# simonsobs/pixell

Measured on AMD Instinct MI355X. Metric: map2alm+alm2map round-trips/sec, higher is better.
Workload: dtype f64

## Files before the change

pixell_amd/csrc/leg_s0.hip:

```cpp
#include "legendre_dev.hpp"

namespace pxs {

#define S0_SYN_PAIR(c0, c1, a0, a1) { \
	PXS_VCOPY(vb0, polar ? c0.c : c0.b); \
	PXS_VCOPY(vb1, polar ? c1.c : c1.b); \
	_Pragma("unroll") for (int s = 0; s < K; s++) { \
		p1r[s] = fma(lam2[s], a0.a, p1r[s]); p1i[s] = fma(lam2[s], a0.b, p1i[s]); \
		p2r[s] = fma(lam2[s], a0.c, p2r[s]); p2i[s] = fma(lam2[s], a0.d, p2i[s]); \
		lam1[s] = fma(fma(c0.a, csq[s], vb0), lam2[s], lam1[s]); \
	} \
	_Pragma("unroll") for (int s = 0; s < K; s++) { \
		p1r[s] = fma(lam1[s], a1.a, p1r[s]); p1i[s] = fma(lam1[s], a1.b, p1i[s]); \
		p2r[s] = fma(lam1[s], a1.c, p2r[s]); p2i[s] = fma(lam1[s], a1.d, p2i[s]); \
		lam2[s] = fma(fma(c1.a, csq[s], vb1), lam1[s], lam2[s]); \
	} }

template<int K> __global__ __launch_bounds__(64, (K == 4 ? 7 : 1)) void leg_syn_s0(const LegK a)
{
	const int lane = threadIdx.x; int wv, m, bb;
	if (!leg_block(a, wv, m, bb)) return;
	const long row0 = PXS_UNIFORM_LONG(a.row[m]);
	const int nk = (a.lmax - m)/2 + 1;
	const double4_t* __restrict__ coef = a.coef + row0;
// ... 33 lines not shown
#pragma unroll
			for (int s = 0; s < K; s++)
				if (sc[s] < 0 && fabs(lam2[s]) > SC_BIG) {
					lam1[s] *= SC_SMALL; lam2[s] *= SC_SMALL;
					if (++sc[s] == 0) p1r[s] = p1i[s] = p2r[s] = p2i[s] = 0;
				}
		}
#pragma unroll
		for (int s = 0; s < K; s++) if (sc[s] < 0) { p1r[s] = p1i[s] = p2r[s] = p2i[s] = 0; lam1[s] = lam2[s] = 0; }
		double4_t c0 = LDC(coef, k), c1 = LDC(coef, k+1), a0 = LDC(at, k), a1 = LDC(at, k+1);
#ifndef PXS_NO_PHASEC_UNROLL
		while (k + 3 < nk) {
			double4_t n0 = LDC(coef, k+2), n1 = LDC(coef, k+3), m0 = LDC(at, k+2), m1 = LDC(at, k+3);
			S0_SYN_PAIR(c0, c1, a0, a1)
			k += 2;
			c0 = LDC(coef, k+2); c1 = LDC(coef, k+3); a0 = LDC(at, k+2); a1 = LDC(at, k+3);
			S0_SYN_PAIR(n0, n1, m0, m1)
			k += 2;
		}
#endif
		for (; k + 1 < nk; k += 2) {
			const double4_t n0 = LDC(coef, k+2), n1 = LDC(coef, k+3), m0 = LDC(at, k+2), m1 = LDC(at, k+3);
			S0_SYN_PAIR(c0, c1, a0, a1)
			c0 = n0; c1 = n1; a0 = m0; a1 = m1;
		}
		if (k < nk) {
#pragma unroll
			for (int s = 0; s < K; s++) {
				p1r[s] = fma(lam2[s], a0.a, p1r[s]); p1i[s] = fma(lam2[s], a0.b, p1i[s]);
				p2r[s] = fma(lam2[s], a0.c, p2r[s]); p2i[s] = fma(lam2[s], a0.d, p2i[s]);
			}
		}
	}
	double2* __restrict__ out = a.leg + (long)bb*a.leg_bs + (long)m*a.ld;
#pragma unroll
	for (int s = 0; s < K; s++) {
		const int p = (wv*K + s)*64 + lane;
		const bool valid = p < a.npairs;
		const int rn_ = valid ? a.ring_n[p] : -1, rs_ = valid ? a.ring_s[p] : -1;
		const double x_ = valid ? a.cth[p] : 0.0;
		if (rn_ >= 0) out[rn_] = make_double2(p1r[s] + x_*p2r[s], p1i[s] + x_*p2i[s]);
		if (rs_ >= 0) out[rs_] = make_double2(p1r[s] - x_*p2r[s], p1i[s] - x_*p2i[s]);
	}
}

#define S0_ANA_PAIR(c0, c1) { \
	PXS_VCOPY(vb0, polar ? c0.c : c0.b); \
	PXS_VCOPY(vb1, polar ? c1.c : c1.b); \
	double t0 = 0, t1 = 0, t2 = 0, t3 = 0, u0 = 0, u1 = 0, u2 = 0, u3 = 0; \
	_Pragma("unroll") for (int s = 0; s < K; s++) { \
		t0 = fma(lam2[s], d1r[s], t0); t1 = fma(lam2[s], d1i[s], t1); t2 = fma(lam2[s], d2r[s], t2); t3 = fma(lam2[s], d2i[s], t3); \
		lam1[s] = fma(fma(c0.a, csq[s], vb0), lam2[s], lam1[s]); \
	} \
	_Pragma("unroll") for (int s = 0; s < K; s++) { \
		u0 = fma(lam1[s], d1r[s], u0); u1 = fma(lam1[s], d1i[s], u1); u2 = fma(lam1[s], d2r[s], u2); u3 = fma(lam1[s], d2i[s], u3); \
		lam2[s] = fma(fma(c1.a, csq[s], vb1), lam1[s], lam2[s]); \
	} \
	 \
	LEG_RED_PUT(kk, t0, t1, t2, t3) \
	LEG_RED_PUT(kk+1, u0, u1, u2, u3) \
	kk += 2; \
	if (kk == LEG_FSTEPS) { leg_flush(red, pout + 4*kbase, lane, LEG_FSTEPS, a.atomic); kk = 0; kbase = k+2; } }

template<int K> __global__ __launch_bounds__(64) void leg_ana_s0(const LegK a)
{
	PXS_SHARED(double, red);
	const int lane = threadIdx.x; int wv, m, bb;
	if (!leg_block(a, wv, m, bb)) return;
	const long row0 = PXS_UNIFORM_LONG(a.row[m]);
	const int nk = (a.lmax - m)/2 + 1;
	const double4_t* __restrict__ coef = a.coef + row0;
	double* __restrict__ pout = a.part + (long)bb*a.mom_bs + ((long)wv*a.rows_chunk + (row0 - a.rowbase))*4;
	const double2* __restrict__ in = a.leg + (long)bb*a.leg_bs + (long)m*a.ld;
	double csq[K], lam1[K], lam2[K], d1r[K], d1i[K], d2r[K], d2i[K];
	int sc[K];
	bool alive_any = false;
	const bool polar = leg_wave_polar(a, wv, K);
	auto load_data = [&](int s) {
		const int p = (wv*K + s)*64 + lane;
		const bool valid = p < a.npairs;
		const int rn = valid ? a.ring_n[p] : -1, rs = valid ? a.ring_s[p] : -1;
		const double x = valid ? a.cth[p] : 0.0;
		const double2 vn = rn >= 0 ? in[rn] : make_double2(0, 0);
		const double2 vs = rs >= 0 ? in[rs] : make_double2(0, 0);
		d1r[s] = vn.x + vs.x; d1i[s] = vn.y + vs.y;
		d2r[s] = (vn.x - vs.x)*x; d2i[s] = (vn.y - vs.y)*x;
	};
#pragma unroll
	for (int s = 0; s < K; s++) {
		const int p = (wv*K + s)*64 + lane;
		const bool valid = p < a.npairs;
		const double x = valid ? a.cth[p] : 0.0;
		const double sth = valid ? a.sth[p] : 0.0;
		csq[s] = polar ? -sth*sth : x*x;
		const bool alive = valid && ((double)m <= a.lmax*sth + a.ofs);
		lam1[s] = 0; lam2[s] = 0; sc[s] = 0;
		if (alive && a.seed_mode != 2) { double mt; int e; pow_scaled(sth, m, mt, e); to_scaled(mt, e, lam2[s], sc[s]); }
		d1r[s] = d1i[s] = d2r[s] = d2i[s] = 0;
		alive_any |= alive;
	}
	if (!__any(alive_any)) return;
	int k = 0;
	S0_SEEDED_PHASE_A
	k = PXS_UNIFORM_INT(k); coef = (const double4_t*)PXS_UNIFORM_LONG((long)coef);
	PXS_COUNT(1, (long)(nk - k)*K*6 + (a.seed_mode != 2 ? (long)k*K*2 : 0L));
	if (lane == 0 && !a.atomic) a.first[wv*a.nmc + (m - a.m0)] = k + 1;
#pragma unroll
	for (int s = 0; s < K; s++) if (sc[s] == 0) load_data(s);
	int kk = 0, kbase = k;
	while (k + 1 < nk) {
		bool pend = false;
#pragma unroll
		for (int s = 0; s < K; s++) pend |= (sc[s] < 0);
		if (!__any(pend)) break;
		for (int it = 0; it < 2 && k + 1 < nk; it++, k += 2) {
			const double4_t c0 = LDC(coef, k), c1 = LDC(coef, k+1);
			S0_ANA_PAIR(c0, c1)
		}
#pragma unroll
		for (int s = 0; s < K; s++)
			if (sc[s] < 0 && fabs(lam2[s]) > SC_BIG) {
				lam1[s] *= SC_SMALL; lam2[s] *= SC_SMALL;
				if (++sc[s] == 0) load_data(s);
			}
	}
	double4_t c0 = LDC(coef, k), c1 = LDC(coef, k+1);
#ifndef PXS_NO_PHASEC_UNROLL
	while (k + 3 < nk) {
		double4_t n0 = LDC(coef, k+2), n1 = LDC(coef, k+3);
		S0_ANA_PAIR(c0, c1)
		k += 2;
		c0 = LDC(coef, k+2); c1 = LDC(coef, k+3);
		S0_ANA_PAIR(n0, n1)
		k += 2;
	}
#endif
	for (; k + 1 < nk; k += 2) {
		const double4_t n0 = LDC(coef, k+2), n1 = LDC(coef, k+3);
		S0_ANA_PAIR(c0, c1)
		c0 = n0; c1 = n1;
	}
	if (k < nk) {
		double t0 = 0, t1 = 0, t2 = 0, t3 = 0;
#pragma unroll
		for (int s = 0; s < K; s++) { t0 = fma(lam2[s], d1r[s], t0); t1 = fma(lam2[s], d1i[s], t1); t2 = fma(lam2[s], d2r[s], t2); t3 = fma(lam2[s], d2i[s], t3); }
		LEG_RED_PUT(kk, t0, t1, t2, t3)
		kk++;
	}
	if (kk > 0) leg_flush(red, pout + 4*kbase, lane, kk, a.atomic);
}


#if defined(PXS_LAB_MMTIME) && !defined(PXS_HOST_SIM)
__device__ unsigned long long mm_prof[16];
#define MM_T0 long long tprev_ = clock64(); unsigned long long tacc_[14] = {0, 0, 0, 0, 0, 0, 0, 0, 0, 0, 0, 0, 0, 0};
#define MM_TICK(i) { const long long tn_ = clock64(); tacc_[i] += (unsigned long long)(tn_ - tprev_); tprev_ = tn_; }
#define MM_TDUMP if (lane == 0) { for (int i_ = 0; i_ < 14; i_++) atomicAdd(&mm_prof[i_], tacc_[i_]); atomicAdd(&mm_prof[15], 1ull); }
#else
#define MM_T0
#define MM_TICK(i)
#define MM_TDUMP
#endif
template<int NG, int W> __global__ __launch_bounds__(64*W, 4) void leg_ana_s0_mm(const LegK a)
{
	PXS_SHARED(double, sh);
	constexpr int K = 1;
	MM_T0
	double* __restrict__ ptile = sh;
	double* __restrict__ red = sh + W*16*MM_PSTRIDE;
	int* __restrict__ s_kmin = reinterpret_cast<int*>(sh + mm_lds_doubles(NG, W));
	const int tid = threadIdx.x, lane = tid & 63, w = PXS_UNIFORM_INT(tid >> 6);
	int wv, m, bb;
	if (!leg_block(a, wv, m, bb)) return;
	const long row0 = PXS_UNIFORM_LONG(a.row[m]);
	const int nk = (a.lmax - m)/2 + 1;
	const double4_t* __restrict__ coef = a.coef + row0;
	const int pbase = wv*64*W;
	const bool polar = [&] { const double c = a.cth[min(pbase + 64*(w + 1), a.npairs) - 1]; return c*c > PXS_POLAR_COS2; }();
	double csq[K], lam1[K], lam2[K]; int sc[K];
	bool alive;
	{
		const int p = pbase + tid;
		const bool valid = p < a.npairs;
		const double x = valid ? a.cth[p] : 0.0, sth = valid ? a.sth[p] : 0.0;
		csq[0] = polar ? -sth*sth : x*x;
		alive = valid && ((double)m <= a.lmax*sth + a.ofs);
		lam1[0] = 0; lam2[0] = 0; sc[0] = 0;
		if (alive) { double mt; int e; pow_scaled(sth, m, mt, e); to_scaled(mt, e, lam2[0], sc[0]); }
	}
	if (tid == 0) *s_kmin = nk;
	__syncthreads();
	MM_TICK(0)
	int k = 0;
	const bool wave_alive = __any(alive);
	if (wave_alive) { S0_PHASE_A }
	const int kw = wave_alive ? PXS_UNIFORM_INT(k) : nk + 16;
	MM_TICK(1)
	if (lane == 0) atomicMin(s_kmin, kw);
	__syncthreads();
	const int kmin = PXS_UNIFORM_INT(*s_kmin);
	MM_TICK(2)
// ... 212 lines not shown
				pmine[(4*q4 + 0)*MMS_PSTRIDE + lane] = p0; pmine[(4*q4 + 1)*MMS_PSTRIDE + lane] = p1;
				pmine[(4*q4 + 2)*MMS_PSTRIDE + lane] = p2; pmine[(4*q4 + 3)*MMS_PSTRIDE + lane] = p3;
			}
			MM_WAVE_SYNC();
			double av[4];
#pragma unroll
			for (int rb = 0; rb < 4; rb++) av[rb] = pread[16*rb];
			MM_WAVE_SYNC();
			if (k0 + 16 < nk) {
#pragma unroll
				for (int i = 0; i < 32; i++) cf[i] = LDCD(tab, 2L*(k0 + 16) + i);
				load_b(k0 + 16, bnxt);
			}
#pragma unroll
			for (int q = 0; q < 4; q++)
#pragma unroll
				for (int rb = 0; rb < 4; rb++) {
					const double aq = q == 0 ? av[rb] : pread[q*MMS_PSTRIDE + 16*rb];
#pragma unroll
					for (int g = 0; g < NG; g++) acc[g][rb] = mm_mfma(aq, bcur[g][q], acc[g][rb]);
				}
			MM_WAVE_SYNC();
#pragma unroll
			for (int g = 0; g < NG; g++)
#pragma unroll
				for (int q = 0; q < 4; q++) bcur[g][q] = bnxt[g][q];
		}
	}
	const int c = lane & 3;
#pragma unroll
	for (int g = 0; g < NG; g++) {
		const int map = (bb*NG + g)*4 + ((lane & 15) >> 2);
		double* __restrict__ out = reinterpret_cast<double*>(a.leg + (long)(map < a.nmaps ? map : 0)*a.leg_bs + (long)m*a.ld) + (c & 1);
#pragma unroll
		for (int rb = 0; rb < 4; rb++)
#pragma unroll
			for (int r = 0; r < 4; r++) {
				const int p = pbase + 16*rb + 4*r + (lane >> 4);
				const bool valid = p < a.npairs && map < a.nmaps;
				const double v = acc[g][rb][r], o = MMS_XOR2(v);
				const double x = valid ? a.cth[p] : 0.0;
				const double val = c < 2 ? fma(x, o, v) : fma(-x, v, o);
				const int ring = valid ? (c < 2 ? a.ring_n[p] : a.ring_s[p]) : -1;
				if (ring >= 0) out[2*ring] = val;
			}
	}
	PXS_COUNT(0, ntile*(NG*256L + 32L) + (wave_alive ? (long)kw*2 : 0L));
}

void launch_leg_syn_s0(int K, dim3 grid, hipStream_t st, const LegK& a) {
#ifdef PXS_LAB
	if (K == 8) { hipLaunchKernelGGL(leg_syn_s0<8>, grid, dim3(64), 0, st, a); return; }
#endif
	if (K == 2) hipLaunchKernelGGL(leg_syn_s0<2>, grid, dim3(64), 0, st, a);
	else        hipLaunchKernelGGL(leg_syn_s0<4>, grid, dim3(64), 0, st, a);
}
void launch_leg_ana_s0(int K, dim3 grid, size_t lds, hipStream_t st, const LegK& a) {
#ifdef PXS_LAB
	if (K == 12) { hipLaunchKernelGGL(leg_ana_s0<12>, grid, dim3(64), lds, st, a); return; }
#endif
	if (K == 8)      hipLaunchKernelGGL(leg_ana_s0<8>, grid, dim3(64), lds, st, a);
	else if (K == 2) hipLaunchKernelGGL(leg_ana_s0<2>, grid, dim3(64), lds, st, a);
	else             hipLaunchKernelGGL(leg_ana_s0<4>, grid, dim3(64), lds, st, a);
}
void launch_leg_syn_s0_mm(int ng, dim3 grid, hipStream_t st, const LegK& a) {
	if (ng == 2) hipLaunchKernelGGL(leg_syn_s0_mm<2>, grid, dim3(64), mm_syn_lds(), st, a);
	else         hipLaunchKernelGGL(leg_syn_s0_mm<1>, grid, dim3(64), mm_syn_lds(), st, a);
}
template<int NG, int W> static void mm_launch1(dim3 grid, hipStream_t st, const LegK& a) {
	static const bool once = [] { (void)hipFuncSetAttribute((const void*)leg_ana_s0_mm<NG, W>, hipFuncAttributeMaxDynamicSharedMemorySize, 160*1024 - 256); return true; }(); (void)once;
	hipLaunchKernelGGL((leg_ana_s0_mm<NG, W>), grid, dim3(64*W), mm_ana_lds(NG, W), st, a);
#if defined(PXS_LAB_MMTIME) && !defined(PXS_HOST_SIM)
	{	unsigned long long h[16]; PXS_HIP(hipStreamSynchronize(st)); PXS_HIP(hipMemcpyFromSymbol(h, HIP_SYMBOL(mm_prof), sizeof(h)));
		static const char* nm_[14] = {"init", "phaseA", "kmin_barrier", "B_final_barriers", "P_phase", "mfma+ds_add", "barrier", "flush", "B_index", "B_data_loads", "B_lds_write+barrier", "B_lds_read", "-", "-"};
		double tot = 0; for (int i = 0; i < 14; i++) tot += (double)h[i];
		fprintf(stderr, "[mm_prof] waves %llu, cycles per wave %.0f:", h[15], tot/std::max(1.0, (double)h[15]));
		for (int i = 0; i < 12; i++) fprintf(stderr, " %s %.1f%%", nm_[i], 100.0*h[i]/tot);
		fprintf(stderr, "\n"); memset(h, 0, sizeof(h)); PXS_HIP(hipMemcpyToSymbol(HIP_SYMBOL(mm_prof), h, sizeof(h))); }
#endif
}
template<int W> static void mm_launch(int ng, dim3 grid, hipStream_t st, const LegK& a) { if (ng == 2) mm_launch1<2, W>(grid, st, a); else mm_launch1<1, W>(grid, st, a); }
void launch_leg_ana_s0_mm(int ng, int W, dim3 grid, hipStream_t st, const LegK& a) {
#ifdef PXS_LAB
	if (W == 16) { mm_launch<16>(ng, grid, st, a); return; }
	if (W == 4)  { mm_launch<4>(ng, grid, st, a); return; }
	if (W == 2)  { mm_launch<2>(ng, grid, st, a); return; }
#endif
	mm_launch<MM_WAVES>(ng, grid, st, a);
}

}
```

pixell_amd/csrc/leg_spin.hip:

```cpp
#include "legendre_dev.hpp"

namespace pxs {

template<int K> struct SpinState {
	double x[K], gp1[K], gp2[K], gm1[K], gm2[K];
	int scp[K], scm[K];
};

template<int K> __device__ __forceinline__ bool spin_init(const LegK& a, int wv, int lane, int m, SpinState<K>& S, int* rn, int* rs, bool polar) {
	const int s_ = a.spin;
	bool alive_any = false;
#pragma unroll
	for (int s = 0; s < K; s++) {
		const int p = (wv*K + s)*64 + lane;
		const bool valid = p < a.npairs;
		rn[s] = valid ? a.ring_n[p] : -1; rs[s] = valid ? a.ring_s[p] : -1;
		const double cth = valid ? a.cth[p] : 0.0;
		const double sth = valid ? a.sth[p] : 0.0;
		const double shh = valid ? a.sh2[p] : 0.0;
		S.x[s] = polar ? -2.0*shh*shh : cth;
		const double t1 = a.lmax*sth + a.ofs;
		const double b = -2.0*s_*fabs(cth);
		const double c = (double)s_*s_ - t1*t1;
		const double discr = b*b - 4*c;
// ... 119 lines not shown
			SPIN_SYN_PAIR(f0, f1, a0, a1)
			j += 2;
			f0 = LDC(coef, j+2); f1 = LDC(coef, j+3); a0 = LDC(at, j+2); a1 = LDC(at, j+3);
			SPIN_SYN_PAIR(n0, n1, m0, m1)
			j += 2;
		}
#endif
		for (; j + 1 < nl; j += 2) {
			const double4_t n0 = LDC(coef, j+2), n1 = LDC(coef, j+3), m0 = LDC(at, j+2), m1 = LDC(at, j+3);
			SPIN_SYN_PAIR(f0, f1, a0, a1)
			f0 = n0; f1 = n1; a0 = m0; a1 = m1;
		}
		if (j < nl) {
#pragma unroll
			for (int s = 0; s < K; s++) {
				const double gp = S.gp2[s], gm = S.gm2[s];
				pnr[s] = fma(gp, a0.a, pnr[s]); pni[s] = fma(gp, a0.b, pni[s]);
				mnr[s] = fma(gm, a0.c, mnr[s]); mni[s] = fma(gm, a0.d, mni[s]);
				qsr[s] = fma(gm, a0.a, qsr[s]); qsi[s] = fma(gm, a0.b, qsi[s]);
				nsr[s] = fma(gp, a0.c, nsr[s]); nsi[s] = fma(gp, a0.d, nsi[s]);
			}
		}
	}
#pragma unroll
	for (int s = 0; s < K; s++) {
		const int p = (wv*K + s)*64 + lane;
		const int rn_ = p < a.npairs ? a.ring_n[p] : -1, rs_ = p < a.npairs ? a.ring_s[p] : -1;
		if (rn_ >= 0) {
			outq[rn_] = make_double2(0.5*(pnr[s] + mnr[s]), 0.5*(pni[s] + mni[s]));
			outu[rn_] = make_double2(0.5*(pni[s] - mni[s]), -0.5*(pnr[s] - mnr[s]));
		}
		if (rs_ >= 0) {
			const double psr = sg0*qsr[s], psi = sg0*qsi[s], msr = sg0*nsr[s], msi = sg0*nsi[s];
			outq[rs_] = make_double2(0.5*(psr + msr), 0.5*(psi + msi));
			outu[rs_] = make_double2(0.5*(psi - msi), -0.5*(psr - msr));
		}
	}
}

#define SPIN_ANA_PAIR(f0, f1) { \
	double t0 = 0, t1 = 0, t2 = 0, t3 = 0, u0 = 0, u1 = 0, u2 = 0, u3 = 0; \
	{ \
		const double ca = f0.a, c1 = polar ? f0.c : f0.b, c2 = polar ? f0.d : -f0.b; \
		PXS_VCOPY(v1, c1); PXS_VCOPY(v2, c2); \
		_Pragma("unroll") for (int s = 0; s < K; s++) { \
			const double gp = S.gp2[s], gm = S.gm2[s]; \
			t0 = fma(gp, tpnr[s], t0); t0 = fma(gm, tpsr[s], t0); \
			t1 = fma(gp, tpni[s], t1); t1 = fma(gm, tpsi[s], t1); \
			t2 = fma(gm, tmnr[s], t2); t2 = fma(gp, tmsr[s], t2); \
			t3 = fma(gm, tmni[s], t3); t3 = fma(gp, tmsi[s], t3); \
			S.gp1[s] = fma(fma(ca, S.x[s], v1), gp, -S.gp1[s]); S.gm1[s] = fma(fma(ca, S.x[s], v2), gm, -S.gm1[s]); \
		} \
	} \
	{ \
		const double ca = f1.a, c1 = polar ? f1.c : f1.b, c2 = polar ? f1.d : -f1.b; \
		PXS_VCOPY(v1, c1); PXS_VCOPY(v2, c2); \
		_Pragma("unroll") for (int s = 0; s < K; s++) { \
			const double gp = S.gp1[s], gm = S.gm1[s]; \
			u0 = fma(gp, tpnr[s], u0); u0 = fma(-gm, tpsr[s], u0); \
			u1 = fma(gp, tpni[s], u1); u1 = fma(-gm, tpsi[s], u1); \
			u2 = fma(gm, tmnr[s], u2); u2 = fma(-gp, tmsr[s], u2); \
			u3 = fma(gm, tmni[s], u3); u3 = fma(-gp, tmsi[s], u3); \
			S.gp2[s] = fma(fma(ca, S.x[s], v1), gp, -S.gp2[s]); S.gm2[s] = fma(fma(ca, S.x[s], v2), gm, -S.gm2[s]); \
		} \
	} \
	 \
	LEG_RED_PUT(kk, t0, t1, t2, t3) \
	LEG_RED_PUT(kk+1, u0, u1, u2, u3) \
	kk += 2; \
	if (kk == LEG_FSTEPS) { leg_flush(red, pout + 4*jbase, lane, LEG_FSTEPS, a.atomic); kk = 0; jbase = j+2; } }

template<int K> __global__ __launch_bounds__(64) void leg_ana_spin(const LegK a)
{
	PXS_SHARED(double, red);
	const int lane = threadIdx.x; int wv, m, bb;
	if (!leg_block(a, wv, m, bb)) return;
	const int l0 = max(m, a.spin);
	const int nl = a.lmax - l0 + 1;
	if (nl <= 0) return;
	const long row0 = PXS_UNIFORM_LONG(a.row[m]);
	const double4_t* __restrict__ coef = a.coef + row0;
	double* __restrict__ pout = a.part + (long)bb*a.mom_bs + ((long)wv*a.rows_chunk + (row0 - a.rowbase))*4;
	const double2* __restrict__ inq = a.leg + (long)bb*a.leg_bs + (long)m*a.ld;
	const double2* __restrict__ inu = a.leg + (long)bb*a.leg_bs + ((long)a.nm + m)*a.ld;
	SpinState<K> S; int rn[K], rs[K];
	const bool polar = leg_wave_polar(a, wv, K);
	const bool alive_any = spin_init<K>(a, wv, lane, m, S, rn, rs, polar);
	if (!__any(alive_any)) return;
	const double sgn0 = ((l0 + m) & 1) ? -1.0 : 1.0;
	double tpnr[K], tpni[K], tmnr[K], tmni[K], tpsr[K], tpsi[K], tmsr[K], tmsi[K];
	auto load_data = [&](int s) {
		const int p = (wv*K + s)*64 + lane;
		const int rn_ = p < a.npairs ? a.ring_n[p] : -1, rs_ = p < a.npairs ? a.ring_s[p] : -1;
		double2 q = rn_ >= 0 ? inq[rn_] : make_double2(0, 0), u = rn_ >= 0 ? inu[rn_] : make_double2(0, 0);
		tpnr[s] = q.x - u.y; tpni[s] = q.y + u.x; tmnr[s] = q.x + u.y; tmni[s] = q.y - u.x;
		q = rs_ >= 0 ? inq[rs_] : make_double2(0, 0); u = rs_ >= 0 ? inu[rs_] : make_double2(0, 0);
		tpsr[s] = sgn0*(q.x - u.y); tpsi[s] = sgn0*(q.y + u.x); tmsr[s] = sgn0*(q.x + u.y); tmsi[s] = sgn0*(q.y - u.x);
	};
#pragma unroll
	for (int s = 0; s < K; s++) tpnr[s] = tpni[s] = tmnr[s] = tmni[s] = tpsr[s] = tpsi[s] = tmsr[s] = tmsi[s] = 0;
	int j = 0;
	SPIN_SEEDED_PHASE_A
	j = PXS_UNIFORM_INT(j); coef = (const double4_t*)PXS_UNIFORM_LONG((long)coef);
	PXS_COUNT(1, (long)(nl - j)*K*12 + (a.seed_mode != 2 ? (long)j*K*4 : 0L));
	if (lane == 0 && !a.atomic) a.first[wv*a.nmc + (m - a.m0)] = j + 1;
#pragma unroll
	for (int s = 0; s < K; s++) if (S.scp[s] == 0 && S.scm[s] == 0) load_data(s);
	int kk = 0, jbase = j;
	while (j + 1 < nl) {
		bool pend = false;
#pragma unroll
		for (int s = 0; s < K; s++) pend |= (S.scp[s] < 0) || (S.scm[s] < 0);
		if (!__any(pend)) break;
		for (int it = 0; it < 2 && j + 1 < nl; it++, j += 2) {
			const double4_t f0 = LDC(coef, j), f1 = LDC(coef, j+1);
			SPIN_ANA_PAIR(f0, f1)
		}
#pragma unroll
		for (int s = 0; s < K; s++) {
			const bool was = (S.scp[s] < 0) || (S.scm[s] < 0);
			if (S.scp[s] < 0 && fabs(S.gp2[s]) > SC_BIG) { S.gp1[s] *= SC_SMALL; S.gp2[s] *= SC_SMALL; S.scp[s]++; }
			if (S.scm[s] < 0 && fabs(S.gm2[s]) > SC_BIG) { S.gm1[s] *= SC_SMALL; S.gm2[s] *= SC_SMALL; S.scm[s]++; }
			if (was && S.scp[s] == 0 && S.scm[s] == 0) load_data(s);
		}
	}
	double4_t f0 = LDC(coef, j), f1 = LDC(coef, j+1);
#ifndef PXS_NO_PHASEC_UNROLL
	while (j + 3 < nl) {
		double4_t n0 = LDC(coef, j+2), n1 = LDC(coef, j+3);
		SPIN_ANA_PAIR(f0, f1)
		j += 2;
		f0 = LDC(coef, j+2); f1 = LDC(coef, j+3);
		SPIN_ANA_PAIR(n0, n1)
		j += 2;
	}
#endif
	for (; j + 1 < nl; j += 2) {
		const double4_t n0 = LDC(coef, j+2), n1 = LDC(coef, j+3);
		SPIN_ANA_PAIR(f0, f1)
		f0 = n0; f1 = n1;
	}
	if (j < nl) {
		double t0 = 0, t1 = 0, t2 = 0, t3 = 0;
#pragma unroll
		for (int s = 0; s < K; s++) {
			const double gp = S.gp2[s], gm = S.gm2[s];
			t0 = fma(gp, tpnr[s], t0); t0 = fma(gm, tpsr[s], t0);
			t1 = fma(gp, tpni[s], t1); t1 = fma(gm, tpsi[s], t1);
			t2 = fma(gm, tmnr[s], t2); t2 = fma(gp, tmsr[s], t2);
			t3 = fma(gm, tmni[s], t3); t3 = fma(gp, tmsi[s], t3);
		}
		LEG_RED_PUT(kk, t0, t1, t2, t3)
		kk++;
	}
	if (kk > 0) leg_flush(red, pout + 4*jbase, lane, kk, a.atomic);
}


struct SpinChain { double x, g1, g2, sgl, pa; int sc; };
__device__ __forceinline__ bool spin_chain_init(const LegK& a, int p, int m, int half, bool polar, SpinChain& C) {
	const int s_ = a.spin;
	const bool valid = p < a.npairs;
	const double cth = valid ? a.cth[p] : 0.0, sth = valid ? a.sth[p] : 0.0, shh = valid ? a.sh2[p] : 0.0;
	C.x = polar ? -2.0*shh*shh : cth; C.sgl = half ? -1.0 : 1.0; C.pa = polar ? 1.0 : 0.0;
	const double t1 = a.lmax*sth + a.ofs, b = -2.0*s_*fabs(cth), c = (double)s_*s_ - t1*t1, discr = b*b - 4*c;
	const double mlim = discr <= 0 ? a.lmax : fmin((double)a.lmax, 0.5*(-b + sqrt(discr)));
	const bool alive = valid && ((double)m <= mlim + 0.5);
	C.g1 = 0; C.g2 = 0; C.sc = 0;
	if (alive) {
		const double sh = shh, ch = a.ch2[p];
		double m1, m2; int e1, e2;
		const int es = m >= s_ ? (half ? m - s_ : m + s_) : (half ? s_ - m : s_ + m), ec = m >= s_ ? (half ? m + s_ : m - s_) : (half ? s_ + m : s_ - m);
		pow_scaled(sh, es, m1, e1); pow_scaled(ch, ec, m2, e2);
		double mt = m1*m2; int e = e1 + e2 + (m >= s_ ? m : 0); frexp_norm(mt, e); to_scaled(mt, e, C.g2, C.sc);
		if (m < s_ && half && ((s_ - m) & 1)) C.g2 = -C.g2;
	}
	return alive;
}
__device__ __forceinline__ double spin_chain_coef(const SpinChain& C, double ca, double cb) { return fma(ca, C.x, fma(C.sgl, cb, C.pa*ca)); }

template<int NG, int W> __global__ __launch_bounds__(64*W, 4) void leg_ana_spin_mm(const LegK a)
{
	PXS_SHARED(double, sh);
	double* __restrict__ ptile = sh;
	double* __restrict__ red = sh + W*16*MM_PSTRIDE;
	int* __restrict__ s_kmin = reinterpret_cast<int*>(sh + mm_lds_doubles(NG, W));
	const int tid = threadIdx.x, lane = tid & 63, w = PXS_UNIFORM_INT(tid >> 6), half = lane >> 5;
	int wv, m, bb;
	if (!leg_block(a, wv, m, bb)) return;
	const int l0 = max(m, a.spin);
	const int nl = a.lmax - l0 + 1;
	if (nl <= 0) return;
	const long row0 = PXS_UNIFORM_LONG(a.row[m]);
	const int pbase = wv*32*W;
	const bool polar = [&] { const double c = a.cth[min(pbase + 32*(w + 1), a.npairs) - 1]; return c*c > PXS_POLAR_COS2; }();
	const int pmine_ = pbase + 32*w + (lane & 31);
	SpinChain C;
	const bool alive = spin_chain_init(a, pmine_, m, half, polar, C);
	const double* __restrict__ tab = reinterpret_cast<const double*>(a.coef2) + 2*row0;
	if (tid == 0) *s_kmin = nl;
	__syncthreads();
	int k = 0;
	const bool wave_alive = __any(alive);
	if (wave_alive) {
		while (k + 4 <= nl) {
			if (__any(C.sc == 0 && C.g2 != 0.0)) break;
			double cq[8];
// ... 229 lines not shown
			double av[4];
#pragma unroll
			for (int rb = 0; rb < 4; rb++) av[rb] = pread[16*rb];
			MM_WAVE_SYNC();
			if (k0 + 16 < nl) {
#pragma unroll
				for (int i = 0; i < 32; i++) cf[i] = LDCD(tab, 2L*(k0 + 16) + i);
				load_b(k0 + 16, bnxt);
			}
#pragma unroll
			for (int q = 0; q < 4; q++)
#pragma unroll
				for (int rb = 0; rb < 4; rb++) {
					const double aq = q == 0 ? av[rb] : pread[q*MMS_PSTRIDE + 16*rb];
#pragma unroll
					for (int g = 0; g < NG; g++) acc[g][rb] = mm_mfma(aq, bcur[g][q], acc[g][rb]);
				}
			MM_WAVE_SYNC();
#pragma unroll
			for (int g = 0; g < NG; g++)
#pragma unroll
				for (int q = 0; q < 4; q++) bcur[g][q] = bnxt[g][q];
		}
	}
	const int c = lane & 3;
#pragma unroll
	for (int g = 0; g < NG; g++) {
		const int map = (bb*NG + g)*4 + ((lane & 15) >> 2);
		double* __restrict__ outq = reinterpret_cast<double*>(a.leg + (long)(map < a.nmaps ? map : 0)*a.leg_bs + (long)m*a.ld);
		double* __restrict__ outu = reinterpret_cast<double*>(a.leg + (long)(map < a.nmaps ? map : 0)*a.leg_bs + ((long)a.nm + m)*a.ld);
#pragma unroll
		for (int rb = 0; rb < 2; rb++)
#pragma unroll
			for (int r = 0; r < 4; r++) {
				const int p = pbase + 16*rb + 4*r + (lane >> 4);
				const bool valid = p < a.npairs && map < a.nmaps;
				const double own = acc[g][rb][r], oth = MMS_XOR2(acc[g][rb + 2][r]);
				const double P = c < 2 ? own : oth, M = c < 2 ? oth : own;
				const double sum = 0.5*(P + M), dif = 0.5*(P - M);
				const int ring = valid ? (c < 2 ? a.ring_n[p] : a.ring_s[p]) : -1;
				if (ring >= 0) {
					if (c & 1) { outq[2*ring + 1] = sum; outu[2*ring] = dif; }
					else       { outq[2*ring] = sum; outu[2*ring + 1] = -dif; }
				}
			}
	}
	PXS_COUNT(0, ntile*(NG*256L + 32L) + (wave_alive ? (long)kw*2 : 0L));
}

void launch_leg_syn_spin(int K, dim3 grid, hipStream_t st, const LegK& a) {
#ifdef PXS_LAB
	if (K == 4) { hipLaunchKernelGGL(leg_syn_spin<4>, grid, dim3(64), 0, st, a); return; }
#endif
	if (K == 3) hipLaunchKernelGGL(leg_syn_spin<3>, grid, dim3(64), 0, st, a);
	else        hipLaunchKernelGGL(leg_syn_spin<2>, grid, dim3(64), 0, st, a);
}
void launch_leg_ana_spin(int K, dim3 grid, size_t lds, hipStream_t st, const LegK& a) {
#ifdef PXS_LAB
	if (K >= 6) { hipLaunchKernelGGL(leg_ana_spin<6>, grid, dim3(64), lds, st, a); return; }
	if (K == 5) { hipLaunchKernelGGL(leg_ana_spin<5>, grid, dim3(64), lds, st, a); return; }
#endif
	if (K >= 4)      hipLaunchKernelGGL(leg_ana_spin<4>, grid, dim3(64), lds, st, a);
	else if (K == 3) hipLaunchKernelGGL(leg_ana_spin<3>, grid, dim3(64), lds, st, a);
	else             hipLaunchKernelGGL(leg_ana_spin<2>, grid, dim3(64), lds, st, a);
}
void launch_leg_syn_spin_mm(int ng, dim3 grid, hipStream_t st, const LegK& a) {
	if (ng == 2) hipLaunchKernelGGL(leg_syn_spin_mm<2>, grid, dim3(64), mm_syn_lds(), st, a);
	else         hipLaunchKernelGGL(leg_syn_spin_mm<1>, grid, dim3(64), mm_syn_lds(), st, a);
}
void launch_leg_ana_spin_mm(int ng, dim3 grid, hipStream_t st, const LegK& a) {
	constexpr int W = MM_WAVES;
	static const bool once = [] { (void)hipFuncSetAttribute((const void*)leg_ana_spin_mm<2, W>, hipFuncAttributeMaxDynamicSharedMemorySize, 160*1024 - 256);
		(void)hipFuncSetAttribute((const void*)leg_ana_spin_mm<1, W>, hipFuncAttributeMaxDynamicSharedMemorySize, 160*1024 - 256); return true; }(); (void)once;
	if (ng == 2) hipLaunchKernelGGL((leg_ana_spin_mm<2, W>), grid, dim3(64*W), mm_ana_lds(2, W), st, a);
	else         hipLaunchKernelGGL((leg_ana_spin_mm<1, W>), grid, dim3(64*W), mm_ana_lds(1, W), st, a);
}

}
```

pixell_amd/csrc/legendre_dev.hpp:

```cpp
#pragma once
#include "legendre.hpp"
#include <cmath>
#include <algorithm>

namespace pxs {

static constexpr double SC_BIG   = 0x1p+400;
static constexpr double SC_SMALL = 0x1p-800;
static constexpr int    SC_STEP  = 800;

struct double4_t { double a, b, c, d; };
#ifdef PXS_HOST_SIM
#define LDC(p, i) ((p)[i])
#else
typedef double pxs_d4 __attribute__((ext_vector_type(4)));
__device__ __forceinline__ double4_t ldc_row(const double4_t* p, long i) {
	const __attribute__((address_space(4))) pxs_d4* c = (const __attribute__((address_space(4))) pxs_d4*)(unsigned long long)p;
	const pxs_d4 v = c[i]; double4_t r; r.a = v.x; r.b = v.y; r.c = v.z; r.d = v.w; return r;
}
#define LDC(p, i) ldc_row((p), (i))
#endif
#ifdef PXS_HOST_SIM
#define LDCD(p, i) ((p)[i])
#else
// ... 94 lines not shown
		S0_PHASE_A \
		if (a.seed_mode == 1) { \
			double* sd = a.seed_d + ((long)m*a.nwave + wv)*(2*K*64); int* si = a.seed_i + ((long)m*a.nwave + wv)*((K+1)*64); \
			_Pragma("unroll") for (int s = 0; s < K; s++) { sd[s*64 + lane] = lam1[s]; sd[(K+s)*64 + lane] = lam2[s]; si[s*64 + lane] = sc[s]; } \
			if (lane == 0) si[K*64] = k; \
		} \
	}
#define SPIN_SEEDED_PHASE_A \
	if (a.seed_mode == 2) { \
		const double* sd = a.seed_d + ((long)m*a.nwave + wv)*(4*K*64); const int* si = a.seed_i + ((long)m*a.nwave + wv)*((2*K+1)*64); \
		j = PXS_UNIFORM_INT(si[2*K*64]); \
		_Pragma("unroll") for (int s = 0; s < K; s++) { \
			S.gp1[s] = sd[s*64 + lane]; S.gp2[s] = sd[(K+s)*64 + lane]; S.gm1[s] = sd[(2*K+s)*64 + lane]; S.gm2[s] = sd[(3*K+s)*64 + lane]; \
			S.scp[s] = si[s*64 + lane]; S.scm[s] = si[(K+s)*64 + lane]; } \
	} else { \
		SPIN_PHASE_A \
		if (a.seed_mode == 1) { \
			double* sd = a.seed_d + ((long)m*a.nwave + wv)*(4*K*64); int* si = a.seed_i + ((long)m*a.nwave + wv)*((2*K+1)*64); \
			_Pragma("unroll") for (int s = 0; s < K; s++) { \
				sd[s*64 + lane] = S.gp1[s]; sd[(K+s)*64 + lane] = S.gp2[s]; sd[(2*K+s)*64 + lane] = S.gm1[s]; sd[(3*K+s)*64 + lane] = S.gm2[s]; \
				si[s*64 + lane] = S.scp[s]; si[(K+s)*64 + lane] = S.scm[s]; } \
			if (lane == 0) si[2*K*64] = j; \
		} \
	}

#define S0_PHASE_A \
	while (k + 4 <= nk) { \
		bool act = false; \
		_Pragma("unroll") for (int s = 0; s < K; s++) act |= (sc[s] == 0 && lam2[s] != 0.0); \
		if (__any(act)) break; \
		const double4_t q0 = LDC(coef, k), q1 = LDC(coef, k+1), q2 = LDC(coef, k+2), q3 = LDC(coef, k+3); \
		const double b0 = polar ? q0.c : q0.b, b1 = polar ? q1.c : q1.b, b2 = polar ? q2.c : q2.b, b3 = polar ? q3.c : q3.b; \
		_Pragma("unroll") for (int s = 0; s < K; s++) { \
			lam1[s] = fma(fma(q0.a, csq[s], b0), lam2[s], lam1[s]); \
			lam2[s] = fma(fma(q1.a, csq[s], b1), lam1[s], lam2[s]); \
			lam1[s] = fma(fma(q2.a, csq[s], b2), lam2[s], lam1[s]); \
			lam2[s] = fma(fma(q3.a, csq[s], b3), lam1[s], lam2[s]); \
			if (sc[s] < 0 && fabs(lam2[s]) > SC_BIG) { lam1[s] *= SC_SMALL; lam2[s] *= SC_SMALL; sc[s]++; } \
		} \
		k += 4; \
	}


#ifdef PXS_HOST_SIM
#define PXS_WAVE_LDS_SYNC() __syncthreads()
#elif defined(PXS_LDS_NOWAIT)
#define PXS_WAVE_LDS_SYNC() asm volatile("" ::: "memory")
#else
#define PXS_WAVE_LDS_SYNC() asm volatile("s_waitcnt lgkmcnt(0)" ::: "memory")
#endif
#define LEG_FSTEPS 16
#ifdef PXS_HOST_SIM
#define LEG_RED_STRIDE 66
#define LEG_RED_DOUBLES (4*LEG_FSTEPS*LEG_RED_STRIDE)
__device__ __forceinline__ double leg_flush_sum(const double* red, int lane) {
	const double* r = red + lane*LEG_RED_STRIDE;
	double s0 = 0, s1 = 0, s2 = 0, s3 = 0;
	for (int i = 0; i < 64; i += 4) { s0 += r[i]; s1 += r[i+1]; s2 += r[i+2]; s3 += r[i+3]; }
	return (s0 + s1) + (s2 + s3);
}
__device__ __forceinline__ int leg_flush_col(int lane) { return lane; }
#define LEG_RED_PUT(kk, t0, t1, t2, t3) \
	red[((kk)*4+0)*LEG_RED_STRIDE + lane] = t0; red[((kk)*4+1)*LEG_RED_STRIDE + lane] = t1; \
	red[((kk)*4+2)*LEG_RED_STRIDE + lane] = t2; red[((kk)*4+3)*LEG_RED_STRIDE + lane] = t3;
#else
#define LEG_RED_STRIDE 18
#define LEG_RED_DOUBLES (4*LEG_FSTEPS*LEG_RED_STRIDE)
__device__ __forceinline__ void leg_swap32(double& a, double& b) {
	const unsigned alo = __double2loint(a), ahi = __double2hiint(a), blo = __double2loint(b), bhi = __double2hiint(b);
	const auto r0 = __builtin_amdgcn_permlane32_swap(alo, blo, false, false);
	const auto r1 = __builtin_amdgcn_permlane32_swap(ahi, bhi, false, false);
	a = __hiloint2double(r1[0], r0[0]); b = __hiloint2double(r1[1], r0[1]);
}
__device__ __forceinline__ void leg_swap16(double& a, double& b) {
	const unsigned alo = __double2loint(a), ahi = __double2hiint(a), blo = __double2loint(b), bhi = __double2hiint(b);
	const auto r0 = __builtin_amdgcn_permlane16_swap(alo, blo, false, false);
	const auto r1 = __builtin_amdgcn_permlane16_swap(ahi, bhi, false, false);
	a = __hiloint2double(r1[0], r0[0]); b = __hiloint2double(r1[1], r0[1]);
}
__device__ __forceinline__ double leg_flush_sum(const double* red, int lane) {
	const double2* r = reinterpret_cast<const double2*>(red + lane*LEG_RED_STRIDE);
	double sum = 0;
#pragma unroll 1
	for (int h = 0; h < 8; h += 4) {
		const double2 a = r[h], b = r[h+1], c = r[h+2], d = r[h+3];
		sum += ((a.x + a.y) + (b.x + b.y)) + ((c.x + c.y) + (d.x + d.y));
	}
	return sum;
}
__device__ __forceinline__ int leg_flush_col(int lane) { const int r = lane & 3; return (lane & ~3) | ((r == 1) ? 2 : (r == 2) ? 1 : r); }
#ifdef PXS_EXP_NORED
#define LEG_RED_PUT(kk, t0, t1, t2, t3) { asm volatile("" :: "v"(t0), "v"(t1), "v"(t2), "v"(t3)); }
#else
#define LEG_RED_PUT(kk, t0, t1, t2, t3) { \
	double a_ = t0, b_ = t1, c_ = t2, d_ = t3; \
	leg_swap32(a_, b_); leg_swap32(c_, d_); \
	double u_ = a_ + b_, v_ = c_ + d_; \
	leg_swap16(u_, v_); \
	red[((kk)*4 + (lane >> 4))*LEG_RED_STRIDE + (lane & 15)] = u_ + v_; }
#endif
#endif
__device__ __forceinline__ void leg_flush(double* red, double* __restrict__ dst, int lane, int nkk, int atomic) {
#if defined(PXS_EXP_NORED) || defined(PXS_EXP_NOFLUSH)
	return;
#endif
	PXS_WAVE_LDS_SYNC();
	if (lane < 4*nkk) {
		const double sum = leg_flush_sum(red, lane);
		double* q = dst + leg_flush_col(lane);
#ifdef PXS_HOST_SIM
		if (atomic) atomicAdd(q, sum); else *q = sum;
#else
		if (atomic) unsafeAtomicAdd(q, sum); else *q = sum;
#endif
	}
	PXS_WAVE_LDS_SYNC();
}


#define MM_PSTRIDE 65
#define MM_WAVES 8
#define MM_ESTRIDE 17
#ifdef PXS_HOST_SIM
struct mm_acc { double v[4]; double& operator[](int i) { return v[i]; } };
static inline mm_acc mm_mfma(double av, double bv, mm_acc c) {
	pxsim::BlockCtx* cx = pxsim::t_ctx; const int w = pxsim::wave_id(), l = pxsim::lane_id();
	uint64_t* s = cx->wslot->data() + (size_t)w*128;
	memcpy(&s[l], &av, 8); memcpy(&s[64 + l], &bv, 8); cx->wbar[w]->wait();
	for (int r = 0; r < 4; r++) {
		const int i = 4*r + (l >> 4), j = l & 15;
		double sum = c.v[r];
		for (int kk = 0; kk < 4; kk++) { double x, y; memcpy(&x, &s[i + 16*kk], 8); memcpy(&y, &s[64 + j + 16*kk], 8); sum = fma(x, y, sum); }
		c.v[r] = sum;
	}
	cx->wbar[w]->wait();
	return c;
}
static inline void mm_lds_add(double* p, double v) { atomicAdd(p, v); }
#define MM_WAVE_SYNC() pxsim::t_ctx->wbar[pxsim::wave_id()]->wait()
#else
typedef double mm_acc __attribute__((ext_vector_type(4)));
__device__ __forceinline__ mm_acc mm_mfma(double av, double bv, mm_acc c) { return __builtin_amdgcn_mfma_f64_16x16x4f64(av, bv, c, 0, 0, 0); }
#ifdef PXS_LAB_NOLDSADD
__device__ __forceinline__ void mm_lds_add(double* p, double v) { *p = v; }
#else
__device__ __forceinline__ void mm_lds_add(double* p, double v) { (void)__hip_atomic_fetch_add(p, v, __ATOMIC_RELAXED, __HIP_MEMORY_SCOPE_WORKGROUP); }
#endif
#define MM_WAVE_SYNC() asm volatile("s_waitcnt lgkmcnt(0)" ::: "memory")
#endif
__device__ __forceinline__ double mm_coef(double ca, double x2, double cb) { PXS_VCOPY(vb_, cb); return fma(ca, x2, vb_); }
__host__ __device__ constexpr int mm_lds_doubles(int NG, int W) { return W*16*MM_PSTRIDE + 2*NG*4*64 > 64*W*MM_ESTRIDE ? W*16*MM_PSTRIDE + 2*NG*4*64 : 64*W*MM_ESTRIDE; }
static inline size_t mm_ana_lds(int NG, int W) { return sizeof(double)*(size_t)mm_lds_doubles(NG, W) + 16; }

#define MMS_PSTRIDE 68
// ... 22 lines not shown
```

Measured before the change: 3.124.

## Software-pipeline analysis reduction cross-half exchange via ds_bpermute overlapping next step

Replaces the synchronous permlane32 swap in the per-step wave reduction with asynchronous ds_bpermute exchanges that are issued after one half-step and consumed one step later. The wait is tied to the recurrence registers so the LDS permute latency overlaps the next block of FMAs. The upper 32 lanes pre-swap their input data pairs so that the exchange needs only two values instead of two swaps. The reduction buffer gains an offset slot because the pipeline starts at kk=-1. The K=8 s0 analysis kernel gets an occupancy hint, and the launchers now reject unsupported K. This adds code complexity and extra registers for the held values, which could cost occupancy.

```diff
diff --git a/pixell_amd/csrc/leg_s0.hip b/pixell_amd/csrc/leg_s0.hip
--- a/pixell_amd/csrc/leg_s0.hip
+++ b/pixell_amd/csrc/leg_s0.hip
@@ -109,19 +109,24 @@
 		t0 = fma(lam2[s], d1r[s], t0); t1 = fma(lam2[s], d1i[s], t1); t2 = fma(lam2[s], d2r[s], t2); t3 = fma(lam2[s], d2i[s], t3); \
 		lam1[s] = fma(fma(c0.a, csq[s], vb0), lam2[s], lam1[s]); \
 	} \
+	 \
+	{ LEG_RED_RECV(hold, r_, t0, t1, t2, t3) LEG_RED_PUT(kk, r_) } kk++; \
+	if (kk == LEG_FSTEPS) { leg_flush(red, pout + 4*kbase, lane, LEG_FSTEPS, a.atomic); kk = 0; kbase += LEG_FSTEPS; } \
+	LEG_RED_SEND(hold, t0, t1, t2, t3) \
+	_Pragma("unroll") for (int s = 0; s < K; s++) { LEG_RED_TIE(lam1[s]); } \
 	_Pragma("unroll") for (int s = 0; s < K; s++) { \
 		u0 = fma(lam1[s], d1r[s], u0); u1 = fma(lam1[s], d1i[s], u1); u2 = fma(lam1[s], d2r[s], u2); u3 = fma(lam1[s], d2i[s], u3); \
 		lam2[s] = fma(fma(c1.a, csq[s], vb1), lam1[s], lam2[s]); \
 	} \
 	 \
-	LEG_RED_PUT(kk, t0, t1, t2, t3) \
-	LEG_RED_PUT(kk+1, u0, u1, u2, u3) \
-	kk += 2; \
-	if (kk == LEG_FSTEPS) { leg_flush(red, pout + 4*kbase, lane, LEG_FSTEPS, a.atomic); kk = 0; kbase = k+2; } }
-
-template<int K> __global__ __launch_bounds__(64) void leg_ana_s0(const LegK a)
+	{ LEG_RED_RECV(hold, r_, u0, u1, u2, u3) LEG_RED_SEND(hold, u0, u1, u2, u3) \
+	  _Pragma("unroll") for (int s = 0; s < K; s++) { LEG_RED_TIE(lam2[s]); } \
+	  LEG_RED_PUT(kk, r_) } kk++; }
+
+template<int K> __global__ __launch_bounds__(64, (K == 8 ? 3 : 1)) void leg_ana_s0(const LegK a)
 {
-	PXS_SHARED(double, red);
+	PXS_SHARED(double, red0);
+	double* red = red0 + 4*LEG_RED_STRIDE;
 	const int lane = threadIdx.x; int wv, m, bb;
 	if (!leg_block(a, wv, m, bb)) return;
 	const long row0 = PXS_UNIFORM_LONG(a.row[m]);
@@ -142,6 +147,7 @@
 		const double2 vs = rs >= 0 ? in[rs] : make_double2(0, 0);
 		d1r[s] = vn.x + vs.x; d1i[s] = vn.y + vs.y;
 		d2r[s] = (vn.x - vs.x)*x; d2i[s] = (vn.y - vs.y)*x;
+		if (LEG_RED_SWAPPED(lane)) { leg_dswap(d1r[s], d1i[s]); leg_dswap(d2r[s], d2i[s]); }
 	};
 #pragma unroll
 	for (int s = 0; s < K; s++) {
@@ -164,7 +170,8 @@
 	if (lane == 0 && !a.atomic) a.first[wv*a.nmc + (m - a.m0)] = k + 1;
 #pragma unroll
 	for (int s = 0; s < K; s++) if (sc[s] == 0) load_data(s);
-	int kk = 0, kbase = k;
+	int kk = -1, kbase = k;
+	LegRedHold hold; LEG_RED_INIT(hold, lane)
 	while (k + 1 < nk) {
 		bool pend = false;
 #pragma unroll
@@ -201,9 +208,11 @@
 		double t0 = 0, t1 = 0, t2 = 0, t3 = 0;
 #pragma unroll
 		for (int s = 0; s < K; s++) { t0 = fma(lam2[s], d1r[s], t0); t1 = fma(lam2[s], d1i[s], t1); t2 = fma(lam2[s], d2r[s], t2); t3 = fma(lam2[s], d2i[s], t3); }
-		LEG_RED_PUT(kk, t0, t1, t2, t3)
-		kk++;
-	}
+		{ LEG_RED_RECV(hold, r_, t0, t1, t2, t3) LEG_RED_PUT(kk, r_) } kk++;
+		if (kk == LEG_FSTEPS) { leg_flush(red, pout + 4*kbase, lane, LEG_FSTEPS, a.atomic); kk = 0; kbase += LEG_FSTEPS; }
+		LEG_RED_SEND(hold, t0, t1, t2, t3)
+	}
+	{ LEG_RED_RECV0(hold, r_) LEG_RED_PUT(kk, r_) } kk++;
 	if (kk > 0) leg_flush(red, pout + 4*kbase, lane, kk, a.atomic);
 }
 
@@ -522,6 +531,7 @@
 #ifdef PXS_LAB
 	if (K == 8) { hipLaunchKernelGGL(leg_syn_s0<8>, grid, dim3(64), 0, st, a); return; }
 #endif
+	PXS_REQUIRE(K == 2 || K == 4, "leg_syn_s0: this build has no kernel for that many ring pairs per lane");
 	if (K == 2) hipLaunchKernelGGL(leg_syn_s0<2>, grid, dim3(64), 0, st, a);
 	else        hipLaunchKernelGGL(leg_syn_s0<4>, grid, dim3(64), 0, st, a);
 }
@@ -529,6 +539,7 @@
 #ifdef PXS_LAB
 	if (K == 12) { hipLaunchKernelGGL(leg_ana_s0<12>, grid, dim3(64), lds, st, a); return; }
 #endif
+	PXS_REQUIRE(K == 8 || K == 4 || K == 2, "leg_ana_s0: this build has no kernel for that many ring pairs per lane");
 	if (K == 8)      hipLaunchKernelGGL(leg_ana_s0<8>, grid, dim3(64), lds, st, a);
 	else if (K == 2) hipLaunchKernelGGL(leg_ana_s0<2>, grid, dim3(64), lds, st, a);
 	else             hipLaunchKernelGGL(leg_ana_s0<4>, grid, dim3(64), lds, st, a);
diff --git a/pixell_amd/csrc/leg_spin.hip b/pixell_amd/csrc/leg_spin.hip
--- a/pixell_amd/csrc/leg_spin.hip
+++ b/pixell_amd/csrc/leg_spin.hip
@@ -195,6 +195,11 @@
 			S.gp1[s] = fma(fma(ca, S.x[s], v1), gp, -S.gp1[s]); S.gm1[s] = fma(fma(ca, S.x[s], v2), gm, -S.gm1[s]); \
 		} \
 	} \
+	 \
+	{ LEG_RED_RECV(hold, r_, t0, t1, t2, t3) LEG_RED_PUT(kk, r_) } kk++; \
+	if (kk == LEG_FSTEPS) { leg_flush(red, pout + 4*jbase, lane, LEG_FSTEPS, a.atomic); kk = 0; jbase += LEG_FSTEPS; } \
+	LEG_RED_SEND(hold, t0, t1, t2, t3) \
+	_Pragma("unroll") for (int s = 0; s < K; s++) { LEG_RED_TIE(S.gp1[s]); LEG_RED_TIE(S.gm1[s]); } \
 	{ \
 		const double ca = f1.a, c1 = polar ? f1.c : f1.b, c2 = polar ? f1.d : -f1.b; \
 		PXS_VCOPY(v1, c1); PXS_VCOPY(v2, c2); \
@@ -208,14 +213,14 @@
 		} \
 	} \
 	 \
-	LEG_RED_PUT(kk, t0, t1, t2, t3) \
-	LEG_RED_PUT(kk+1, u0, u1, u2, u3) \
-	kk += 2; \
-	if (kk == LEG_FSTEPS) { leg_flush(red, pout + 4*jbase, lane, LEG_FSTEPS, a.atomic); kk = 0; jbase = j+2; } }
+	{ LEG_RED_RECV(hold, r_, u0, u1, u2, u3) LEG_RED_SEND(hold, u0, u1, u2, u3) \
+	  _Pragma("unroll") for (int s = 0; s < K; s++) { LEG_RED_TIE(S.gp2[s]); LEG_RED_TIE(S.gm2[s]); } \
+	  LEG_RED_PUT(kk, r_) } kk++; }
 
 template<int K> __global__ __launch_bounds__(64) void leg_ana_spin(const LegK a)
 {
-	PXS_SHARED(double, red);
+	PXS_SHARED(double, red0);
+	double* red = red0 + 4*LEG_RED_STRIDE;
 	const int lane = threadIdx.x; int wv, m, bb;
 	if (!leg_block(a, wv, m, bb)) return;
 	const int l0 = max(m, a.spin);
@@ -239,6 +244,7 @@
 		tpnr[s] = q.x - u.y; tpni[s] = q.y + u.x; tmnr[s] = q.x + u.y; tmni[s] = q.y - u.x;
 		q = rs_ >= 0 ? inq[rs_] : make_double2(0, 0); u = rs_ >= 0 ? inu[rs_] : make_double2(0, 0);
 		tpsr[s] = sgn0*(q.x - u.y); tpsi[s] = sgn0*(q.y + u.x); tmsr[s] = sgn0*(q.x + u.y); tmsi[s] = sgn0*(q.y - u.x);
+		if (LEG_RED_SWAPPED(lane)) { leg_dswap(tpnr[s], tpni[s]); leg_dswap(tmnr[s], tmni[s]); leg_dswap(tpsr[s], tpsi[s]); leg_dswap(tmsr[s], tmsi[s]); }
 	};
 #pragma unroll
 	for (int s = 0; s < K; s++) tpnr[s] = tpni[s] = tmnr[s] = tmni[s] = tpsr[s] = tpsi[s] = tmsr[s] = tmsi[s] = 0;
@@ -249,7 +255,8 @@
 	if (lane == 0 && !a.atomic) a.first[wv*a.nmc + (m - a.m0)] = j + 1;
 #pragma unroll
 	for (int s = 0; s < K; s++) if (S.scp[s] == 0 && S.scm[s] == 0) load_data(s);
-	int kk = 0, jbase = j;
+	int kk = -1, jbase = j;
+	LegRedHold hold; LEG_RED_INIT(hold, lane)
 	while (j + 1 < nl) {
 		bool pend = false;
 #pragma unroll
@@ -293,9 +300,11 @@
 			t2 = fma(gm, tmnr[s], t2); t2 = fma(gp, tmsr[s], t2);
 			t3 = fma(gm, tmni[s], t3); t3 = fma(gp, tmsi[s], t3);
 		}
-		LEG_RED_PUT(kk, t0, t1, t2, t3)
-		kk++;
-	}
+		{ LEG_RED_RECV(hold, r_, t0, t1, t2, t3) LEG_RED_PUT(kk, r_) } kk++;
+		if (kk == LEG_FSTEPS) { leg_flush(red, pout + 4*jbase, lane, LEG_FSTEPS, a.atomic); kk = 0; jbase += LEG_FSTEPS; }
+		LEG_RED_SEND(hold, t0, t1, t2, t3)
+	}
+	{ LEG_RED_RECV0(hold, r_) LEG_RED_PUT(kk, r_) } kk++;
 	if (kk > 0) leg_flush(red, pout + 4*jbase, lane, kk, a.atomic);
 }
 
@@ -631,15 +640,17 @@
 #ifdef PXS_LAB
 	if (K == 4) { hipLaunchKernelGGL(leg_syn_spin<4>, grid, dim3(64), 0, st, a); return; }
 #endif
+	PXS_REQUIRE(K == 3 || K == 2, "leg_syn_spin: this build has no kernel for that many ring pairs per lane");
 	if (K == 3) hipLaunchKernelGGL(leg_syn_spin<3>, grid, dim3(64), 0, st, a);
 	else        hipLaunchKernelGGL(leg_syn_spin<2>, grid, dim3(64), 0, st, a);
 }
 void launch_leg_ana_spin(int K, dim3 grid, size_t lds, hipStream_t st, const LegK& a) {
 #ifdef PXS_LAB
-	if (K >= 6) { hipLaunchKernelGGL(leg_ana_spin<6>, grid, dim3(64), lds, st, a); return; }
+	if (K == 6) { hipLaunchKernelGGL(leg_ana_spin<6>, grid, dim3(64), lds, st, a); return; }
 	if (K == 5) { hipLaunchKernelGGL(leg_ana_spin<5>, grid, dim3(64), lds, st, a); return; }
 #endif
-	if (K >= 4)      hipLaunchKernelGGL(leg_ana_spin<4>, grid, dim3(64), lds, st, a);
+	PXS_REQUIRE(K >= 2 && K <= 4, "leg_ana_spin: this build has no kernel for that many ring pairs per lane");
+	if (K == 4)      hipLaunchKernelGGL(leg_ana_spin<4>, grid, dim3(64), lds, st, a);
 	else if (K == 3) hipLaunchKernelGGL(leg_ana_spin<3>, grid, dim3(64), lds, st, a);
 	else             hipLaunchKernelGGL(leg_ana_spin<2>, grid, dim3(64), lds, st, a);
 }
diff --git a/pixell_amd/csrc/legendre_dev.hpp b/pixell_amd/csrc/legendre_dev.hpp
--- a/pixell_amd/csrc/legendre_dev.hpp
+++ b/pixell_amd/csrc/legendre_dev.hpp
@@ -170,7 +170,7 @@
 #define LEG_FSTEPS 16
 #ifdef PXS_HOST_SIM
 #define LEG_RED_STRIDE 66
-#define LEG_RED_DOUBLES (4*LEG_FSTEPS*LEG_RED_STRIDE)
+#define LEG_RED_DOUBLES (4*(LEG_FSTEPS + 1)*LEG_RED_STRIDE)
 __device__ __forceinline__ double leg_flush_sum(const double* red, int lane) {
 	const double* r = red + lane*LEG_RED_STRIDE;
 	double s0 = 0, s1 = 0, s2 = 0, s3 = 0;
@@ -178,18 +178,19 @@
 	return (s0 + s1) + (s2 + s3);
 }
 __device__ __forceinline__ int leg_flush_col(int lane) { return lane; }
-#define LEG_RED_PUT(kk, t0, t1, t2, t3) \
-	red[((kk)*4+0)*LEG_RED_STRIDE + lane] = t0; red[((kk)*4+1)*LEG_RED_STRIDE + lane] = t1; \
-	red[((kk)*4+2)*LEG_RED_STRIDE + lane] = t2; red[((kk)*4+3)*LEG_RED_STRIDE + lane] = t3;
+struct LegRedHold { double t[4]; };
+#define LEG_RED_INIT(h, lane) { h.t[0] = h.t[1] = h.t[2] = h.t[3] = 0; }
+#define LEG_RED_SWAPPED(lane) false
+#define LEG_RED_SEND(h, t0, t1, t2, t3) { h.t[0] = t0; h.t[1] = t1; h.t[2] = t2; h.t[3] = t3; }
+#define LEG_RED_TIE(x)
+#define LEG_RED_RECV(h, r, a0, a1, a2, a3) const LegRedHold r = h;
+#define LEG_RED_RECV0(h, r) const LegRedHold r = h;
+#define LEG_RED_PUT(kk, r) { \
+	red[((kk)*4+0)*LEG_RED_STRIDE + lane] = r.t[0]; red[((kk)*4+1)*LEG_RED_STRIDE + lane] = r.t[1]; \
+	red[((kk)*4+2)*LEG_RED_STRIDE + lane] = r.t[2]; red[((kk)*4+3)*LEG_RED_STRIDE + lane] = r.t[3]; }
 #else
 #define LEG_RED_STRIDE 18
-#define LEG_RED_DOUBLES (4*LEG_FSTEPS*LEG_RED_STRIDE)
-__device__ __forceinline__ void leg_swap32(double& a, double& b) {
-	const unsigned alo = __double2loint(a), ahi = __double2hiint(a), blo = __double2loint(b), bhi = __double2hiint(b);
-	const auto r0 = __builtin_amdgcn_permlane32_swap(alo, blo, false, false);
-	const auto r1 = __builtin_amdgcn_permlane32_swap(ahi, bhi, false, false);
-	a = __hiloint2double(r1[0], r0[0]); b = __hiloint2double(r1[1], r0[1]);
-}
+#define LEG_RED_DOUBLES (4*(LEG_FSTEPS + 1)*LEG_RED_STRIDE)
 __device__ __forceinline__ void leg_swap16(double& a, double& b) {
 	const unsigned alo = __double2loint(a), ahi = __double2hiint(a), blo = __double2loint(b), bhi = __double2hiint(b);
 	const auto r0 = __builtin_amdgcn_permlane16_swap(alo, blo, false, false);
@@ -207,17 +208,35 @@
 	return sum;
 }
 __device__ __forceinline__ int leg_flush_col(int lane) { const int r = lane & 3; return (lane & ~3) | ((r == 1) ? 2 : (r == 2) ? 1 : r); }
+struct LegRedHold { double k0, k2; int r1l, r1h, r3l, r3h; int xaddr; };
+#define LEG_RED_INIT(h, lane) { h.k0 = h.k2 = 0; h.r1l = h.r1h = h.r3l = h.r3h = 0; h.xaddr = ((lane) ^ 32) << 2; }
+#define LEG_RED_SWAPPED(lane) ((lane) >= 32)
+struct LegRedSum { double u, v; };
+#define LEG_RED_TIE(x) asm volatile("" : "+v"(x))
 #ifdef PXS_EXP_NORED
-#define LEG_RED_PUT(kk, t0, t1, t2, t3) { asm volatile("" :: "v"(t0), "v"(t1), "v"(t2), "v"(t3)); }
-#else
-#define LEG_RED_PUT(kk, t0, t1, t2, t3) { \
-	double a_ = t0, b_ = t1, c_ = t2, d_ = t3; \
-	leg_swap32(a_, b_); leg_swap32(c_, d_); \
-	double u_ = a_ + b_, v_ = c_ + d_; \
+#define LEG_RED_SEND(h, t0, t1, t2, t3) { asm volatile("" :: "v"(t0), "v"(t1), "v"(t2), "v"(t3)); }
+#define LEG_RED_RECV(h, r, a0, a1, a2, a3)
+#define LEG_RED_RECV0(h, r)
+#define LEG_RED_PUT(kk, r) { }
+#else
+#define LEG_RED_SEND(h, t0, t1, t2, t3) { \
+	h.k0 = t0; h.k2 = t2; \
+	asm volatile("ds_bpermute_b32 %0, %4, %5\n\tds_bpermute_b32 %1, %4, %6\n\tds_bpermute_b32 %2, %4, %7\n\tds_bpermute_b32 %3, %4, %8" \
+		: "=&v"(h.r1l), "=&v"(h.r1h), "=&v"(h.r3l), "=&v"(h.r3h) \
+		: "v"(h.xaddr), "v"(__double2loint(t1)), "v"(__double2hiint(t1)), "v"(__double2loint(t3)), "v"(__double2hiint(t3))); }
+#define LEG_RED_RECV(h, r, a0, a1, a2, a3) \
+	asm volatile("s_waitcnt lgkmcnt(0)" : "+v"(h.r1l), "+v"(h.r1h), "+v"(h.r3l), "+v"(h.r3h), "+v"(a0), "+v"(a1), "+v"(a2), "+v"(a3)); \
+	LegRedSum r; r.u = h.k0 + __hiloint2double(h.r1h, h.r1l); r.v = h.k2 + __hiloint2double(h.r3h, h.r3l);
+#define LEG_RED_RECV0(h, r) \
+	asm volatile("s_waitcnt lgkmcnt(0)" : "+v"(h.r1l), "+v"(h.r1h), "+v"(h.r3l), "+v"(h.r3h)); \
+	LegRedSum r; r.u = h.k0 + __hiloint2double(h.r1h, h.r1l); r.v = h.k2 + __hiloint2double(h.r3h, h.r3l);
+#define LEG_RED_PUT(kk, r) { \
+	double u_ = r.u, v_ = r.v; \
 	leg_swap16(u_, v_); \
 	red[((kk)*4 + (lane >> 4))*LEG_RED_STRIDE + (lane & 15)] = u_ + v_; }
 #endif
 #endif
+__device__ __forceinline__ void leg_dswap(double& a, double& b) { const double t = a; a = b; b = t; }
 __device__ __forceinline__ void leg_flush(double* red, double* __restrict__ dst, int lane, int nkk, int atomic) {
 #if defined(PXS_EXP_NORED) || defined(PXS_EXP_NOFLUSH)
 	return;
```

New measurement: 3.086. -1.2%, worse.
